# qingpingmo/OCN

Measured on AMD Instinct MI355X. Metric: candidate-edges/sec (CN predictor fwd), ogbl-collab shape, higher is better.
Workload: dtype f32

## Files before the change

include/ocn_hip.h:

```cpp
#ifndef OCN_HIP_H
#define OCN_HIP_H

#include <stdint.h>

#ifdef __cplusplus
extern "C" {
#endif

#define OCN_ABI_VERSION 9
#define OCN_EINVAL (-1)
#define OCN_ECAP   (-2)

#define OCN_ST_CAP  1
#define OCN_ST_SCAN 2
#define OCN_SCAN_POISON (-1)

#define OCN_F_CN1 1u
#define OCN_F_CN2 2u

int ocn_abi_version(void);

int64_t ocn_scan_workspace_bytes(int64_t n);

int ocn_zero_regions(void* const* ptrs, const int64_t* bytes, int32_t n, void* stream);
// ... 25 lines not shown
                    int64_t B, int64_t* order_out, int64_t* inv_out, int64_t* ranges, int64_t* prefix,
                    void* workspace, void* stream);

int ocn_scan_i32(const int32_t* in, int64_t n, int64_t* out, void* workspace, void* stream);

int ocn_cn_flags(const int64_t* rowptrA, const int32_t* colA,
                 const int64_t* rowptrT1, const int32_t* colT1,
                 const int64_t* rowptrT2, const int32_t* colT2,
                 const uint32_t* bitmapT1 , int64_t bm1_stride_words,
                 const uint32_t* bitmapT2 , int64_t bm_stride_words,
                 const int64_t* src, const int64_t* dst, const int64_t* order, int64_t B,
                 int64_t n_cols, const int64_t* off, uint8_t* flags, int64_t flags_cap,
                 uint64_t* hist , int32_t* cnt1, int32_t* cnt2,
                 int32_t* status, uint64_t* rec , int32_t* gcost , void* stream);
int ocn_cn_flags_rec(const int64_t* rowptrA, const int32_t* colA,
                     const int64_t* rowptrT1, const int32_t* colT1,
                     const int64_t* rowptrT2, const int32_t* colT2,
                     const uint32_t* bitmapT1 , int64_t bm1_stride_words,
                     const uint32_t* bitmapT2 , int64_t bm_stride_words,
                     const int64_t* src, const int64_t* dst, const int64_t* order, int64_t B,
                     int64_t n_cols, const int64_t* off, uint8_t* flags, int64_t flags_cap,
                     uint64_t* hist , int32_t* cnt1, int32_t* cnt2,
                     int32_t* status, uint64_t* rec , int32_t* gcost , void* stream);

int32_t ocn_walk_chunk(void);
int ocn_cn_walk_flags(const int64_t* rowptrA, const int32_t* colA, const int64_t* nds ,
                      const int64_t* src, const int64_t* dst, const int64_t* order, int64_t B,
                      const int64_t* chunk_off, const int64_t* rev_off , const int64_t* off,
                      int64_t max_row_len ,
                      uint8_t* flags, int32_t* wc, int64_t flags_cap,
                      uint64_t* hist , int32_t* cnt1, int32_t* cnt2,
                      int32_t* status, void* stream);

int ocn_neighbor_degree_sum(const int64_t* rowptr, const int32_t* col, int64_t n_rows, int64_t* out,
                            void* stream);
int ocn_walk_rev_offsets(const int64_t* rowptrA, const int64_t* nds, const int64_t* src, const int64_t* dst,
                         const int64_t* order, int64_t B, int64_t* out , void* workspace,
                         void* stream);

int32_t ocn_walk_prep_max_batch(void);
int ocn_walk_prep(const int64_t* rowptrA, const int64_t* nds , const int64_t* src, const int64_t* dst,
                  int64_t B, int32_t min_share, int64_t* order, int64_t* off, int64_t* chunk_off,
                  int64_t* rev_off , int32_t* g_head , int64_t* g_item_off ,
                  int32_t* g_active , int32_t* meta, int32_t* cnt1,
                  int32_t* cnt2, int32_t* status, int32_t* scal, void* stream);
int ocn_cn_walk_group(const int64_t* rowptrA, const int32_t* colA, const int64_t* src, const int64_t* dst,
// ... 332 lines not shown
```

ocn_amd/_lib.py:

```python
from __future__ import annotations

import ctypes
import glob
import os
import subprocess
from ctypes import c_float, c_int32, c_int64, c_void_p

_HERE = os.path.dirname(os.path.abspath(__file__))
_ROOT = os.path.dirname(_HERE)
LIB_PATH = os.environ.get("OCN_LIB_PATH", os.path.join(_HERE, "libocn_hip.so"))
CSRC = os.path.join(_HERE, "csrc")
INCLUDE = os.path.join(_ROOT, "include")

_P = c_void_p
ABI_VERSION = 9
SIGNATURES = {
    "ocn_abi_version": (c_int32, []),
    "ocn_scan_workspace_bytes": (c_int64, [c_int64]),
    "ocn_zero_regions": (c_int32, [_P, _P, c_int32, _P]),
    "ocn_check_edges": (c_int32, [_P, _P, c_int64, c_int64, c_int64, _P, _P]),
    "ocn_edge_offsets": (c_int32, [_P, _P, c_int64, _P, _P, _P]),
    "ocn_class_order": (c_int32, [_P, _P, _P, c_int64, _P, _P, _P, _P, _P, _P]),
    "ocn_scan_i32": (c_int32, [_P, c_int64, _P, _P, _P]),
    "ocn_order_workspace_bytes": (c_int64, [c_int64]),
    "ocn_order_by_node": (c_int32, [_P, c_int64, c_int64, _P, _P, _P]),
    "ocn_order_by_node_finish": (c_int32, [_P, c_int64, c_int64, _P, _P, _P]),
    "ocn_order_by_node_finish_rec": (c_int32, [_P, _P, _P, _P, c_int64, c_int64, _P, _P, _P, _P]),
    "ocn_batch_prep": (c_int32, [_P, _P, c_int64, _P, _P, c_int64, _P, _P, _P, c_int32, _P]),
    "ocn_cn_flags": (c_int32, [_P, _P, _P, _P, _P, _P, _P, c_int64, _P, c_int64, _P, _P, _P, c_int64, c_int64, _P, _P, c_int64, _P,
                               _P, _P, _P, _P, _P, _P]),
    "ocn_cn_flags_rec": (c_int32, [_P, _P, _P, _P, _P, _P, _P, c_int64, _P, c_int64, _P, _P, _P, c_int64, c_int64, _P, _P, c_int64, _P,
                                   _P, _P, _P, _P, _P, _P]),
    "ocn_chunk_offsets": (c_int32, [_P, _P, _P, _P, c_int64, _P, _P, _P]),
    "ocn_walk_chunk": (c_int32, []),
    "ocn_cn_walk_flags": (c_int32, [_P, _P, _P, _P, _P, _P, c_int64, _P, _P, _P, c_int64, _P, _P, c_int64, _P, _P, _P,
                                    _P, _P]),
    "ocn_neighbor_degree_sum": (c_int32, [_P, _P, c_int64, _P, _P]),
    "ocn_walk_prep_max_batch": (c_int32, []),
    "ocn_cn_flags_small_graph_cols": (c_int32, []),
    "ocn_cn_flags_pair_min_batch": (c_int64, [c_int64]),
    "ocn_walk_prep": (c_int32, [_P, _P, _P, _P, c_int64, c_int32, _P, _P, _P, _P, _P, _P, _P, _P, _P, _P, _P, _P, _P]),
    "ocn_cn_walk_group": (c_int32, [_P, _P, _P, _P, _P, c_int64, _P, _P, _P, _P, _P, _P, _P, c_int64, _P, _P, _P, _P]),
    "ocn_walk_rev_offsets": (c_int32, [_P, _P, _P, _P, _P, c_int64, _P, _P, _P]),
    "ocn_cn_weights_cn5": (c_int32, [_P, c_int64, _P, _P, c_int32, _P, _P]),
    "ocn_cn5_column_stats": (c_int32, [_P, c_int64, _P, _P]),
    "ocn_cn_colsum_workspace_bytes": (c_int64, [c_int64, c_int64]),
    "ocn_cn_colsum_exact": (c_int32, [_P, _P, _P, c_int64, _P, _P, _P, _P, c_int64, _P, c_int64, _P, _P, _P, _P, _P, _P, _P]),
    "ocn_cn_weights_cn7": (c_int32, [_P, c_int64, c_float, _P, _P, _P]),
    "ocn_cn_gather": (c_int32, [_P, _P, _P, _P, _P, c_int64, _P, _P, _P, _P, _P, c_int32, c_int64, _P, _P, _P, _P, _P,
                                _P, _P, _P, _P, _P]),
    "ocn_cn8_pool": (c_int32, [_P, _P, _P, _P, _P, _P, _P, c_int64, _P, c_int64, _P, _P, _P, c_int64, c_int64, _P, c_int32, _P, _P,
                               _P, _P, _P, _P]),
    "ocn_cn_pool_frozen": (c_int32, [_P, _P, _P, _P, _P, _P, _P, c_int64, _P, c_int64, _P, _P, _P, c_int64, c_int64, _P, _P, c_int32, _P,
                                     _P, _P, _P, _P, _P]),
    "ocn_cn_attribution": (c_int32, [_P, _P, _P, _P, c_int64, _P, _P, _P, c_int64, _P, _P, c_int32, _P, _P, _P, _P, _P]),
# ... 202 lines not shown
```

ocn_amd/csrc/cn_flags.hip:

```cpp
#include "common.h"


__device__ __forceinline__ bool sampled_has(const int32_t* samp, const int32_t* __restrict__ row, i64 n,
                                            int32_t key) {
  int lo = 0, hi = OCN_WAVE;
  while (lo < hi) {
    const int mid = (lo + hi) >> 1;
    if (samp[mid] <= key) lo = mid + 1; else hi = mid;
  }
  if (lo == 0) return false;
  const int s = lo - 1;
  const i64 p0 = ((i64)s * n) >> 6, p1 = ((i64)(s + 1) * n) >> 6;
  return sorted_has(row + p0, p1 - p0, key);
}

#define T1_CAP 1024

#define LH_MAX_COLS 8192

__device__ __forceinline__ i64 wave_uniform(i64 v) {
  const unsigned lo = __builtin_amdgcn_readfirstlane((unsigned)(u64)v), hi = __builtin_amdgcn_readfirstlane((unsigned)((u64)v >> 32));
  return (i64)(((u64)hi << 32) | lo);
}
__device__ __forceinline__ bool lanes_have(int32_t t, int32_t key) {
  int pos = 0;
#pragma unroll
  for (int step = OCN_WAVE / 2; step > 0; step >>= 1)
    if (__shfl(t, pos + step - 1, OCN_WAVE) < key) pos += step;
  return __shfl(t, pos, OCN_WAVE) == key;
}

template <bool HAS_T2, bool LH, bool RECIN, int NS>
__global__ __launch_bounds__(OCN_BLOCK) void cn_flags_kernel(
    const i64* __restrict__ rowptrA, const int32_t* __restrict__ colA,
    const i64* __restrict__ rowptrT1, const int32_t* __restrict__ colT1,
    const i64* __restrict__ rowptrT2, const int32_t* __restrict__ colT2,
    const unsigned* __restrict__ bmT1, i64 bm1_stride, const unsigned* __restrict__ bmT2, i64 bm_stride,
    const i64* __restrict__ src, const i64* __restrict__ dst, const i64* __restrict__ order, i64 B,
    i64 n_cols, const i64* __restrict__ off, uint8_t* __restrict__ flags, i64 cap,
    u64* __restrict__ hist, int32_t* __restrict__ cnt1, int32_t* __restrict__ cnt2,
    int32_t* __restrict__ status, u64* rec, int32_t* __restrict__ gcost) {
  constexpr int GPB = OCN_WPB, SPB = GPB * NS;
  constexpr int T1_PART = T1_CAP / NS, T2_PART = OCN_WAVE / NS;
  static_assert(NS == 1 || (NS == 2 && !LH), "slot pairs: large-graph forms only");
  __shared__ int s_cost[2][GPB];
  __shared__ int32_t s_t1[GPB][T1_CAP];
  __shared__ int32_t s_t2[GPB][OCN_WAVE];
  extern __shared__ __attribute__((aligned(16))) u64 s_hist[];
  const int gl = threadIdx.x % OCN_WAVE, g = __builtin_amdgcn_readfirstlane(threadIdx.x / OCN_WAVE);
  if (blockIdx.x == 0 && threadIdx.x == 0) status_raise(status, off[B], cap);
  const bool void_batch = off[B] < 0;
  if (LH) {
    for (i64 c = threadIdx.x; c < n_cols; c += OCN_BLOCK) s_hist[c] = 0ull;
    __syncthreads();
  }
  int par = 0;
  for (i64 e0 = (i64)blockIdx.x * SPB; e0 < B; e0 += (i64)gridDim.x * SPB, par ^= 1) {
    i64 slot[NS];
    bool act[NS];
    i64 e[NS], i[NS], j[NS], a0[NS], da[NS], b0[NS], db[NS], c0[NS], dc[NS], base[NS];
    const unsigned* bm_row[NS];
    const unsigned* bm1_row[NS];
#pragma unroll
    for (int s = 0; s < NS; ++s) {
// ... 17 lines not shown
#pragma unroll
            for (int q = 0; q < 4; ++q)
              w[q] = (u64)(unsigned)__builtin_amdgcn_readlane((int)(unsigned)recw, 4 * s + q) |
                     ((u64)(unsigned)__builtin_amdgcn_readlane((int)(unsigned)(recw >> 32), 4 * s + q) << 32);
          }
          e[s] = wave_uniform((i64)w[0]);
          i[s] = wave_uniform((i64)(w[1] & 0xffffffffull)); j[s] = wave_uniform((i64)(w[1] >> 32));
          a0[s] = wave_uniform((i64)(w[2] & ((1ull << REC_LEN_SHIFT) - 1))); da[s] = wave_uniform((i64)(w[2] >> REC_LEN_SHIFT));
          base[s] = wave_uniform((i64)w[3]);
        } else {
          e[s] = order ? order[slot[s]] : slot[s];
          i[s] = src[e[s]]; j[s] = dst[e[s]];
          a0[s] = rowptrA[i[s]]; da[s] = rowptrA[i[s] + 1] - a0[s];
          base[s] = off[e[s]];
        }
        if (bmT1) bm1_row[s] = bmT1 + j[s] * bm1_stride;
        else { b0[s] = rowptrT1[j[s]]; db[s] = rowptrT1[j[s] + 1] - b0[s]; }
        if (HAS_T2) {
          if (bmT2) bm_row[s] = bmT2 + j[s] * bm_stride;
          if (rowptrT2 && (LH || !bmT2)) { c0[s] = rowptrT2[j[s]]; dc[s] = rowptrT2[j[s] + 1] - c0[s]; }
        }
        if (void_batch) { da[s] = 0; db[s] = 0; dc[s] = 0; base[s] = 0; }
      }
    bool t1_reg[NS], t1_lds[NS], t2_full[NS], t2_lds[NS];
    int t1_at[NS], t2_at[NS];
    int32_t t1[NS];
#pragma unroll
    for (int s = 0; s < NS; ++s) {
      const int o = (s + 1) % NS;
      const bool whole1 = NS == 1 || db[o] <= OCN_WAVE;
      t1_reg[s] = db[s] <= OCN_WAVE; t1_lds[s] = db[s] <= (whole1 ? T1_CAP : T1_PART);
      t1_at[s] = whole1 ? 0 : s * T1_PART;
      t1[s] = 0x7fffffff;
      if (t1_reg[s]) { if (gl < db[s]) t1[s] = colT1[b0[s] + gl]; }
      else if (t1_lds[s])
        for (i64 q = gl; q < db[s]; q += OCN_WAVE) s_t1[g][t1_at[s] + q] = colT1[b0[s] + q];
    }
#pragma unroll
    for (int s = 0; s < NS; ++s) {
      const int o = (s + 1) % NS;
      t2_full[s] = HAS_T2 && rowptrT2 && dc[s] == n_cols;
      const bool whole2 = NS == 1 || (HAS_T2 && rowptrT2 && dc[o] == n_cols) || dc[o] == 0;
      t2_lds[s] = whole2 || dc[s] <= T2_PART;
      t2_at[s] = whole2 ? 0 : s * T2_PART;
      if (HAS_T2 && !t2_full[s] && !bmT2 && t2_lds[s]) {
        if (dc[s] > OCN_WAVE) s_t2[g][gl] = colT2[c0[s] + (((i64)gl * dc[s]) >> 6)];
        else if (gl < dc[s]) s_t2[g][t2_at[s] + gl] = colT2[c0[s] + gl];
      }
    }
    wave_lds_sync();
    bool fits[NS];
    int c1[NS], c2[NS];
    i64 da_max = da[0];
#pragma unroll
    for (int s = 0; s < NS; ++s) {
      fits[s] = base[s] + da[s] <= cap;
      c1[s] = c2[s] = 0;
      if (s > 0 && da[s] > da_max) da_max = da[s];
    }
    const bool same = NS > 1 && i[0] == i[NS - 1];
    for (i64 p0 = 0; p0 < da_max; p0 += OCN_WAVE) {
      const i64 p = p0 + gl;
      bool in[NS], f1[NS], f2[NS];
      int32_t k[NS];
      unsigned w2[NS];
#pragma unroll
      for (int s = 0; s < NS; ++s) {
        in[s] = p < da[s];
        if (s > 0 && same) k[s] = k[0];
        else k[s] = in[s] ? colA[a0[s] + p] : 0;
      }
#pragma unroll
      for (int s = 0; s < NS; ++s) {
        w2[s] = 0;
        if (HAS_T2 && bmT2 && !t2_full[s] && in[s]) w2[s] = bm_row[s][k[s] >> 5];
      }
#pragma unroll
      for (int s = 0; s < NS; ++s) {
        if (bmT1) f1[s] = in[s] && ((bm1_row[s][k[s] >> 5] >> (k[s] & 31)) & 1u);
        else if (t1_reg[s]) f1[s] = lanes_have(t1[s], k[s]) && in[s];
        else f1[s] = in[s] && (t1_lds[s] ? sorted_has(&s_t1[g][t1_at[s]], db[s], k[s]) : sorted_has(colT1 + b0[s], db[s], k[s]));
      }
#pragma unroll
      for (int s = 0; s < NS; ++s) {
        f2[s] = false;
        if (HAS_T2 && in[s]) {
          if (t2_full[s]) f2[s] = true;
          else if (bmT2) f2[s] = (w2[s] >> (k[s] & 31)) & 1u;
          else if (!t2_lds[s]) f2[s] = sorted_has(colT2 + c0[s], dc[s], k[s]);
          else f2[s] = dc[s] > OCN_WAVE ? sampled_has(&s_t2[g][0], colT2 + c0[s], dc[s], k[s]) : sorted_has(&s_t2[g][t2_at[s]], dc[s], k[s]);
        }
        if (fits[s] && in[s]) flags[base[s] + p] = (uint8_t)((f1[s] ? OCN_F_CN1 : 0u) | (f2[s] ? OCN_F_CN2 : 0u));
      }
      if (NS > 1 && same) {
        u64 inc = 0;
#pragma unroll
        for (int s = 0; s < NS; ++s) inc += (u64)f1[s] | ((u64)f2[s] << HF_BITS) | ((u64)(f1[s] | f2[s]) << (2 * HF_BITS));
        if (inc) atomicAdd(hist + 2 * (i64)k[0], inc);
      } else {
#pragma unroll
        for (int s = 0; s < NS; ++s)
          if (f1[s] | f2[s]) {
            const u64 inc = (u64)f1[s] | ((u64)f2[s] << HF_BITS) | (1ull << (2 * HF_BITS));
            if (LH) atomicAdd(s_hist + k[s], inc); else atomicAdd(hist + 2 * (i64)k[s], inc);
          }
      }
#pragma unroll
      for (int s = 0; s < NS; ++s) {
        c1[s] += __popcll(__ballot(f1[s]));
        c2[s] += __popcll(__ballot(f2[s]));
// ... 39 lines not shown
      const u64 v = s_hist[c];
      if (v) atomicAdd(hist + 2 * c, v);
    }
  }
}

extern "C" {

int32_t ocn_cn_flags_small_graph_cols(void) { return LH_MAX_COLS; }

static int64_t g_flags_pair_min_batch = 32768;

int64_t ocn_cn_flags_pair_min_batch(int64_t min_rows) {
  const int64_t prev = g_flags_pair_min_batch;
  if (min_rows >= 0) g_flags_pair_min_batch = min_rows;
  return prev;
}

static int cn_flags_launch(const int64_t* rowptrA, const int32_t* colA, const int64_t* rowptrT1,
                           const int32_t* colT1, const int64_t* rowptrT2, const int32_t* colT2,
                           const uint32_t* bitmapT1, int64_t bm1_stride_words, const uint32_t* bitmapT2, int64_t bm_stride_words,
                           const int64_t* src, const int64_t* dst, const int64_t* order, int64_t B,
                           int64_t n_cols, const int64_t* off, uint8_t* flags, int64_t flags_cap, uint64_t* hist,
                           int32_t* cnt1, int32_t* cnt2, int32_t* status, uint64_t* rec, int32_t* gcost, bool rec_in, void* stream) {
  if (B < 0 || flags_cap < 0 || B > (int64_t)HF_MASK) return OCN_EINVAL;
  if (B == 0) return 0;
  if (!rowptrA || (!rowptrT1 && !bitmapT1) || !src || !dst || !off || !hist || !cnt1 || !status) return OCN_EINVAL;
  if (rec_in && (!rec || !order)) return OCN_EINVAL;
  if ((bitmapT1 && bm1_stride_words * 32 < n_cols) || (bitmapT2 && bm_stride_words * 32 < n_cols)) return OCN_EINVAL;
  constexpr int GPB = OCN_WPB;
  hipStream_t st = (hipStream_t)stream;
  const bool lh = n_cols > 0 && n_cols <= LH_MAX_COLS;
  const size_t lds = lh ? (size_t)n_cols * sizeof(u64) : 0;
  const bool pairs = !lh && B >= g_flags_pair_min_batch;
  const int spb = pairs ? 2 * GPB : GPB;
  const int grid = lh ? grid_for((B + GPB - 1) / GPB, 256 * 3) : grid_for((B + spb - 1) / spb);
  if (lh) {
    static bool raised_dev[64] = {};
    int devid = 0;
    if (hipGetDevice(&devid) != hipSuccess || devid < 0 || devid >= 64) return OCN_EINVAL;
    bool& raised = raised_dev[devid];
    if (!raised) {
      const void* fns[4] = {(const void*)cn_flags_kernel<true, true, false, 1>, (const void*)cn_flags_kernel<false, true, false, 1>,
                            (const void*)cn_flags_kernel<true, true, true, 1>, (const void*)cn_flags_kernel<false, true, true, 1>};
      for (const void* fn : fns) {
        hipError_t e1 = hipFuncSetAttribute(fn, hipFuncAttributeMaxDynamicSharedMemorySize, LH_MAX_COLS * (int)sizeof(u64));
        if (e1 != hipSuccess) return (int)e1;
      }
      raised = true;
    }
  }
#define CN_FLAGS_ARGS(T2P, T2C)                                                                      \
  (const i64*)rowptrA, colA, (const i64*)rowptrT1, colT1, (const i64*)(T2P), (T2C),                   \
      (const unsigned*)bitmapT1, (i64)bm1_stride_words, (const unsigned*)bitmapT2, (i64)bm_stride_words, (const i64*)src, \
      (const i64*)dst, (const i64*)order, (i64)B, (i64)n_cols, (const i64*)off, flags, (i64)flags_cap, \
      (u64*)hist, cnt1, cnt2, status, (u64*)rec, gcost
#define CN_FLAGS_LAUNCH(T2, LHV, RI, NSV, T2P, T2C)                                                   \
  hipLaunchKernelGGL((cn_flags_kernel<T2, LHV, RI, NSV>), dim3(grid), dim3(OCN_BLOCK), (LHV) ? lds : 0, st, CN_FLAGS_ARGS(T2P, T2C))
#define CN_FLAGS_PICK(T2, T2P, T2C)                                                                   \
  do {                                                                                                \
    if (lh) { if (rec_in) CN_FLAGS_LAUNCH(T2, true, true, 1, T2P, T2C); else CN_FLAGS_LAUNCH(T2, true, false, 1, T2P, T2C); }   \
    else if (pairs) { if (rec_in) CN_FLAGS_LAUNCH(T2, false, true, 2, T2P, T2C); else CN_FLAGS_LAUNCH(T2, false, false, 2, T2P, T2C); }   \
    else { if (rec_in) CN_FLAGS_LAUNCH(T2, false, true, 1, T2P, T2C); else CN_FLAGS_LAUNCH(T2, false, false, 1, T2P, T2C); }    \
  } while (0)
  if (!rowptrT2 && bitmapT2 && lh) return OCN_EINVAL;
  if (rowptrT2 || bitmapT2) CN_FLAGS_PICK(true, rowptrT2, colT2);
  else CN_FLAGS_PICK(false, nullptr, (const int32_t*)nullptr);
#undef CN_FLAGS_PICK
#undef CN_FLAGS_LAUNCH
  return launch_status();
}

int ocn_cn_flags(const int64_t* rowptrA, const int32_t* colA, const int64_t* rowptrT1,
                 const int32_t* colT1, const int64_t* rowptrT2, const int32_t* colT2,
                 const uint32_t* bitmapT1, int64_t bm1_stride_words, const uint32_t* bitmapT2, int64_t bm_stride_words,
                 const int64_t* src, const int64_t* dst, const int64_t* order, int64_t B,
                 int64_t n_cols, const int64_t* off, uint8_t* flags, int64_t flags_cap, uint64_t* hist,
                 int32_t* cnt1, int32_t* cnt2, int32_t* status, uint64_t* rec, int32_t* gcost, void* stream) {
  return cn_flags_launch(rowptrA, colA, rowptrT1, colT1, rowptrT2, colT2, bitmapT1, bm1_stride_words, bitmapT2, bm_stride_words,
                         src, dst, order, B, n_cols, off, flags, flags_cap, hist, cnt1, cnt2, status, rec, gcost, false, stream);
}

int ocn_cn_flags_rec(const int64_t* rowptrA, const int32_t* colA, const int64_t* rowptrT1,
                     const int32_t* colT1, const int64_t* rowptrT2, const int32_t* colT2,
                     const uint32_t* bitmapT1, int64_t bm1_stride_words, const uint32_t* bitmapT2, int64_t bm_stride_words,
                     const int64_t* src, const int64_t* dst, const int64_t* order, int64_t B,
                     int64_t n_cols, const int64_t* off, uint8_t* flags, int64_t flags_cap, uint64_t* hist,
                     int32_t* cnt1, int32_t* cnt2, int32_t* status, uint64_t* rec, int32_t* gcost, void* stream) {
  return cn_flags_launch(rowptrA, colA, rowptrT1, colT1, rowptrT2, colT2, bitmapT1, bm1_stride_words, bitmapT2, bm_stride_words,
                         src, dst, order, B, n_cols, off, flags, flags_cap, hist, cnt1, cnt2, status, rec, gcost, true, stream);
}

}
```

ocn_amd/ops.py:

```python
from __future__ import annotations

import ctypes
import os
from typing import Optional, Tuple

import torch
from torch import Tensor

from . import _lib
from ._lib import check, ptr, stream_ptr

FLAGS_NOSYNC_LIMIT = 1 << 30
validate_indices = True
stage_timer = None
LN_WIDTHS = (16, 32, 64, 128, 256, 512)
a1_bitmap_max_bytes = int(os.environ.get("OCN_A1_BITMAP_MAX_BYTES", 64 << 20))
a2_bitmap_max_bytes = 16 << 30
skip_zero_rows = True
skip_zero_min_share = 0.15
skip_zero_backoff = 32
skip_zero_min_batch = 4096
walk_two_sided = True
walk_share_min = 2
sort_edges_min_batch = 4096
heavy_first = os.environ.get("OCN_HEAVY_FIRST", "1") != "0"
sched_segment = int(os.environ.get("OCN_SCHED_SEG", 0))
overlap_depth = int(os.environ.get("OCN_OVERLAP_DEPTH", 4))
overlap_depth_small = int(os.environ.get("OCN_OVERLAP_DEPTH_SMALL", 8))
overlap_small_batch = 4096
overlap_deep_max_batch = int(os.environ.get("OCN_OVERLAP_DEEP_MAX_BATCH", 1 << 30))
shard_reduce_in_finish = {"0": False, "1": True}.get(os.environ.get("OCN_REDUCE_IN_FINISH", ""), None)
_overlap_active = False
phase_a_extras = os.environ.get("OCN_PHASE_A_EXTRAS", "1") != "0"
phase_a_pool = os.environ.get("OCN_PHASE_A_POOL", "1") != "0"
graph_loops = os.environ.get("OCN_GRAPH_LOOPS", "0") == "1"
graph_loops_min_batches_per_set = 6
overlap_min_batch = 2048
overlap_streams = os.environ.get("OCN_ONE_STREAM", "0") != "1"
share_full_rows = True
deterministic_backward = os.environ.get("OCN_ATOMIC_BACKWARD", "0") != "1"


def loop_depth(batch) -> int:
    if batch is None or batch > overlap_deep_max_batch:
        return 2
    return max(2, int(overlap_depth_small if batch <= overlap_small_batch else overlap_depth))


# ... 206 lines not shown


def _nds_arg(nds: Optional[Tensor], n: int) -> Optional[Tensor]:
    if nds is not None and _req(nds, torch.int64, "nds", 1).numel() != n:
        raise ValueError("nds does not match the adjacency")
    return nds


def _flag_capacity(B: int, max_deg_a: int, off: Tensor) -> int:
    bound = B * max(int(max_deg_a), 0)
    return bound if bound <= FLAGS_NOSYNC_LIMIT else _total(off[-1])


def _cn_operands(rowptrA, colA, t1, t2, bm1, bm2, src, dst, order, B: int, n_cols: int):
    return (ptr(rowptrA), ptr(colA), ptr(t1[0]), ptr(t1[1]), ptr(t2[0]), ptr(t2[1]),
            ptr(bm1), bm1.shape[1] if bm1 is not None else 0, ptr(bm2), bm2.shape[1] if bm2 is not None else 0,
            ptr(src), ptr(dst), ptr(order), B, n_cols)


@_on_device
def cn_flags(rowptrA: Tensor, colA: Tensor, t1: Optional[Tuple[Tensor, Tensor]],
             t2: Optional[Tuple[Tensor, Tensor]], src: Tensor, dst: Tensor, n_cols: int, max_deg_a: int,
             walk: bool = False, t2_bitmap: Optional[Tensor] = None, wsd=None, nds: Optional[Tensor] = None,
             t1_bitmap: Optional[Tensor] = None, rec: Optional[Tensor] = None, sched: Optional[Tensor] = None):
    dev = src.device
    _req(rowptrA, torch.int64, "rowptrA", 1); _req(colA, torch.int32, "colA", 1)
    has_t2 = not walk and t2 is not None
    if not walk:
        *csr1, rows = _t_of_flag_pass(t1, t1_bitmap, "T1", n_cols)
        if t2 is None and t2_bitmap is not None:
            raise ValueError("t2_bitmap does not match the T2 adjacency")
        *csr2, _ = (None, None, None) if not has_t2 else _t_of_flag_pass(
            t2, t2_bitmap, "T2", n_cols, like=rows, col_deferred=True, rowptr_optional=t2[0] is None and n_cols > small_graph_cols())
    B = _batch_ids(src, dst, hist=True)
    _mark("begin")
    if walk and 0 < B <= int(_lib.lib().ocn_walk_prep_max_batch()) and walk_share_min > 0:
        return _cn_flags_walk_small(rowptrA, colA, src, dst, n_cols, max_deg_a, wsd, nds)
    want_order = B >= sort_edges_min_batch
    n_src = rowptrA.numel() - 1
    order = buf(wsd, "order", B, torch.int64, dev) if want_order else None
    ows = (buf(wsd, "order_ws", int(_lib.lib().ocn_order_workspace_bytes(n_src)) // 8 + 1, torch.int64, dev, zero_init=True)
           if want_order else None)
    off = buf(wsd, "off", B + 1, torch.int64, dev)
    sws = _ws(B, dev, wsd)
    hist = buf(wsd, "hist", (n_cols, 2), torch.int64, dev)
    cnt1 = buf(wsd, "cnt1", B, torch.int32, dev)
    cnt2 = buf(wsd, "cnt2", B, torch.int32, dev) if (walk or has_t2) else None
# ... 18 lines not shown
        check(_lib.lib().ocn_order_by_node_finish(ptr(src), B, n_src, ptr(order), ptr(ows), stream_ptr()),
              "ocn_order_by_node_finish")
    cap = _flag_capacity(B, max_deg_a, off)
    flags = buf(wsd, "flags", max(cap, 1), torch.uint8, dev)
    wc = buf(wsd, "wc", max(cap, 1), torch.int32, dev) if walk else None
    chunk_off = rev_off = None
    if walk:
        nds = _nds_arg(nds if walk_two_sided else None, n_src)
        chunk_off = buf(wsd, "chunk_off", B + 1, torch.int64, dev)
        cws = _ws(B, dev, wsd)
        check(_lib.lib().ocn_chunk_offsets(ptr(rowptrA), ptr(nds), ptr(src), ptr(order), B, ptr(chunk_off), ptr(cws),
                                           stream_ptr()), "ocn_chunk_offsets")
        if nds is not None:
            rev_off = buf(wsd, "rev_off", B + 1, torch.int64, dev)
            check(_lib.lib().ocn_walk_rev_offsets(ptr(rowptrA), ptr(nds), ptr(src), ptr(dst), ptr(order), B,
                                                  ptr(rev_off), ptr(cws), stream_ptr()), "ocn_walk_rev_offsets")
    _mark("cn_prep")
    if walk:
        check(_lib.lib().ocn_cn_walk_flags(ptr(rowptrA), ptr(colA), ptr(nds), ptr(src), ptr(dst), ptr(order), B,
                                           ptr(chunk_off), ptr(rev_off), ptr(off), int(max_deg_a), ptr(flags),
                                           ptr(wc), cap, ptr(hist), ptr(cnt1), ptr(cnt2), ptr(status),
                                           stream_ptr()), "ocn_cn_walk_flags")
    else:
        check((_lib.lib().ocn_cn_flags_rec if rec_in else _lib.lib().ocn_cn_flags)(
            *_cn_operands(rowptrA, colA, csr1, csr2, t1_bitmap, t2_bitmap, src, dst, order, B, n_cols), ptr(off), ptr(flags), cap,
            ptr(hist), ptr(cnt1), ptr(cnt2), ptr(status), ptr(rec), ptr(sched), stream_ptr()), "ocn_cn_flags")
    _mark("cn_flags")
    return order, off, flags, wc, hist, cnt1, cnt2, status, scal


def _cn_flags_walk_small(rowptrA, colA, src, dst, n_cols, max_deg_a, wsd, nds):
    dev, B = src.device, src.numel()
    l = _lib.lib()
    nds = _nds_arg(nds if walk_two_sided else None, rowptrA.numel() - 1)
    order = buf(wsd, "order", B, torch.int64, dev)
    off = buf(wsd, "off", B + 1, torch.int64, dev)
    chunk_off = buf(wsd, "chunk_off", B + 1, torch.int64, dev)
    rev_off = buf(wsd, "rev_off", B + 1, torch.int64, dev) if nds is not None else None
    g_head = buf(wsd, "g_head", B + 1, torch.int32, dev)
    g_item_off = buf(wsd, "g_item_off", B + 1, torch.int64, dev)
    g_active = buf(wsd, "g_active", B, torch.int32, dev)
    meta = buf(wsd, "walk_meta", 4, torch.int32, dev)
    hist = buf(wsd, "hist", (n_cols, 2), torch.int64, dev)
    cnt1 = buf(wsd, "cnt1", B, torch.int32, dev)
    cnt2 = buf(wsd, "cnt2", B, torch.int32, dev)
    status = buf(wsd, "status", 4, torch.int32, dev, zero_init=True)
    scal = buf(wsd, "scal", 4, torch.int32, dev)
    check(l.ocn_walk_prep(ptr(rowptrA), ptr(nds), ptr(src), ptr(dst), B, int(walk_share_min), ptr(order), ptr(off),
                          ptr(chunk_off), ptr(rev_off), ptr(g_head), ptr(g_item_off), ptr(g_active), ptr(meta), ptr(cnt1),
# ... 1659 lines not shown
```

ocn_amd/sparse.py:

```python
from __future__ import annotations

from typing import List, Optional, Tuple

import torch
from torch import Tensor

from . import ops


class _Storage:
    def __init__(self, owner: "SparseTensor"):
        self._o = owner

    def row(self) -> Tensor:
        return self._o._row64()

    def col(self) -> Tensor:
        return self._o._col.to(torch.int64)

    def rowptr(self) -> Tensor:
        return self._o._rowptr

    def rowcount(self) -> Tensor:
        return self._o._rowptr[1:] - self._o._rowptr[:-1]

    def value(self) -> Optional[Tensor]:
        return self._o._value

    def has_value(self) -> bool:
        return self._o._value is not None


class SparseTensor:
    def __new__(cls, row=None, rowptr=None, col=None, value=None, sparse_sizes=None, *a, **k):
        cn = getattr(row, "_ocn_lazy_cn", None)
        if cn is not None:
            if getattr(col, "_ocn_lazy_cn", None) is not cn or (value is not None and getattr(value, "_ocn_lazy_cn", None) is not cn):
                raise NotImplementedError("row / col / value of different deferred common-neighbour matrices")
            if sparse_sizes is not None and tuple(int(v) for v in sparse_sizes) != tuple(cn.shape):
                raise ValueError(f"sparse_sizes {tuple(sparse_sizes)} != {tuple(cn.shape)} of the deferred matrix")
            return cn.batch()
        return super().__new__(cls)

    def __init__(self, row: Optional[Tensor] = None, rowptr: Optional[Tensor] = None,
                 col: Optional[Tensor] = None, value: Optional[Tensor] = None,
                 sparse_sizes: Optional[Tuple[int, int]] = None, is_sorted: bool = False,
                 trust_data: bool = False):
        assert col is not None and (row is not None or rowptr is not None)
        if sparse_sizes is None:
            n_rows = (int(row.max()) + 1 if row.numel() else 0) if rowptr is None else rowptr.numel() - 1
            n_cols = int(col.max()) + 1 if col.numel() else 0
            sparse_sizes = (n_rows, n_cols)
        self._sizes = (int(sparse_sizes[0]), int(sparse_sizes[1]))
        if rowptr is None and value is None and not is_sorted and col.is_cuda:
            rowptr, col = ops.coo_to_csr(row.to(torch.int64), col.to(torch.int64), self._sizes[0], self._sizes[1],
                                         check_range=not trust_data)
# ... 194 lines not shown
        return self._bitmap

    def neighbor_degree_sum(self) -> Tensor:
        if self._nds is None:
            self._nds = ops.neighbor_degree_sum(self._rowptr, self._col)
            self._published("nds")
        else:
            self._await("nds")
        return self._nds

    def product_bit_rows(self) -> Optional[Tensor]:
        self.complete()
        if self._bitmap is not None:
            self._await("bitmap")
        return self._bitmap

    def probed_bit_rows(self, dst: Tensor, row_lengths: bool = False) -> Optional[Tensor]:
        if self.rows_on_demand() and not ops._overlap_active and not (row_lengths and self._sizes[1] <= ops.small_graph_cols()):
            a_rp, a_col, b_rp, b_col = self._lazy
            ops.spgemm_bit_rows(a_rp, a_col, b_rp, b_col, self._sizes[1], dst, self._done, self._bitmap)
            return self._bitmap
        return self.product_bit_rows()

    def rows_on_demand(self) -> bool:
        return getattr(self, "_lazy", None) is not None

    def complete(self) -> None:
        if self.rows_on_demand():
            self._complete()

    def warm(self, walk: bool = False) -> None:
        self.max_rowcount()
        if walk:
            self.neighbor_degree_sum()
        else:
            self.bit_rows()

    def to_device(self, device, non_blocking: bool = False) -> "SparseTensor":
        out = SparseTensor(rowptr=self._rowptr.to(device, non_blocking=non_blocking),
                           col=self._col.to(device, non_blocking=non_blocking),
                           value=None if self._value is None else self._value.to(device, non_blocking=non_blocking),
                           sparse_sizes=self._sizes)
        out._maxdeg = self._maxdeg
        return out

    def to(self, device, non_blocking: bool = False):
        return self.to_device(device, non_blocking)

    def cuda(self):
        return self.to_device("cuda")

    def cpu(self):
        return self.to_device("cpu")

    def set_value(self, value: Optional[Tensor]) -> "SparseTensor":
        out = SparseTensor(rowptr=self._rowptr, col=self._col, value=value, sparse_sizes=self._sizes)
        out._row_cache, out._maxdeg = self._row_cache, self._maxdeg
        return out

    def fill_value(self, v: float, dtype=torch.float32) -> "SparseTensor":
        return self.set_value(torch.full((self.nnz(),), v, dtype=dtype, device=self._col.device))

    def fill_value_(self, v: float, dtype=torch.float32) -> "SparseTensor":
        self._value = torch.full((self.nnz(),), v, dtype=dtype, device=self._col.device)
        return self

    def coalesce(self, reduce: str = "sum") -> "SparseTensor":
        n = max(self._sizes[1], 1)
        key = self._row64() * n + self._col.to(torch.int64)
        if self._value is None:
            ukey = torch.unique_consecutive(key)
            val = None
        else:
            ukey, inv = torch.unique_consecutive(key, return_inverse=True)
            val = torch.zeros(ukey.numel(), dtype=self._value.dtype, device=key.device).index_add_(0, inv, self._value)
        return SparseTensor(row=torch.div(ukey, n, rounding_mode="floor"), col=ukey % n, value=val,
                            sparse_sizes=self._sizes, is_sorted=True, trust_data=True)

    def to_symmetric(self, reduce: str = "sum") -> "SparseTensor":
        r, c = self._row64(), self._col.to(torch.int64)
        if self._value is None and self._col.is_cuda and self._sizes[0] == self._sizes[1]:
            rowptr, col = ops.coo_to_csr(r, c, self._sizes[0], self._sizes[1], symmetrize=True, dedupe=True, check_range=False)
            return SparseTensor(rowptr=rowptr, col=col, sparse_sizes=self._sizes)
        v = None if self._value is None else torch.cat([self._value, self._value])
        return SparseTensor(row=torch.cat([r, c]), col=torch.cat([c, r]), value=v,
                            sparse_sizes=self._sizes, trust_data=True).coalesce(reduce)

    def t(self) -> "SparseTensor":
        if getattr(self, "_t_cache", None) is None:
            r, c = self._row64(), self._col.to(torch.int64)
            self._t_cache = SparseTensor(row=c, col=r, value=self._value, sparse_sizes=(self._sizes[1], self._sizes[0]),
                                         trust_data=True)
        return self._t_cache

    def __getitem__(self, idx: Tensor) -> "SparseTensor":
        idx = idx.to(torch.int64)
        start = self._rowptr[idx]
        deg = self._rowptr[idx + 1] - start
        optr = torch.zeros(idx.numel() + 1, dtype=torch.int64, device=idx.device)
        torch.cumsum(deg, 0, out=optr[1:])
        total = int(optr[-1])
        row = torch.repeat_interleave(torch.arange(idx.numel(), device=idx.device), deg, output_size=total)
        pos = torch.arange(total, device=idx.device) - optr[:-1][row] + start[row]
        return SparseTensor(rowptr=optr, col=self._col[pos],
                            value=None if self._value is None else self._value[pos],
                            sparse_sizes=(idx.numel(), self._sizes[1]))

    def to_dense(self) -> Tensor:
        d = torch.zeros(self._sizes, device=self._col.device)
# ... 55 lines not shown
        self.sp = sp
        self.is_product = is_product

    @property
    def shape(self):
        return tuple(self.sp._sizes)

    def __matmul__(self, other: "CooView") -> "CooView":
        a, b = self.sp, other.sp
        if a._sizes[1] != b._sizes[0]:
            raise ValueError("shape mismatch in sparse @ sparse")
        n, m = a._sizes[0], b._sizes[1]
        if (ops.lazy_product_rows and torch.is_grad_enabled() and a._rowptr.is_cuda and m > ops.small_graph_cols()
                and 0 < n * ((m + 31) // 32) * 4 <= ops.a2_bitmap_max_bytes and m <= ops.spgemm_max_cols()):
            return CooView(SparseTensor._lazy_product(a, b), is_product=True)
        rowptr, col, bitmap = ops.spgemm_pattern(a._rowptr, a._col, b._rowptr, b._col, b._sizes[1], defer_fill=True)
        if callable(col):
            out = SparseTensor._deferred_product(rowptr, col, bitmap, (a._sizes[0], b._sizes[1]))
        else:
            out = SparseTensor(rowptr=rowptr, col=col, sparse_sizes=(a._sizes[0], b._sizes[1]))
            out._bitmap = bitmap
        if bitmap is not None:
            out._published("bitmap")
        return CooView(out, is_product=True)

    def to_torch(self) -> Tensor:
        sp = self.sp
        v = sp._value if sp._value is not None else torch.ones(sp.nnz(), device=sp.device())
        return torch.sparse_coo_tensor(torch.stack([sp._row64(), sp._col.to(torch.int64)]), v, sp._sizes)
```

ocn_amd/update.py:

```python
from __future__ import annotations

import warnings
from typing import List, Optional, Tuple

import torch
import torch.nn as nn
from torch import Tensor

from . import ops
from .sparse import SparseTensor


_WORDS = {"insert_edges": ("new_edges", "take new entries"), "remove_edges": ("edges", "give up entries")}


def _check_args(fn: str, adj: SparseTensor, edges: Tensor, adj2: Optional[SparseTensor]) -> int:
    arg, verb = _WORDS[fn]
    if not isinstance(adj, SparseTensor) or (adj2 is not None and not isinstance(adj2, SparseTensor)):
        raise ValueError(f"{fn}: adj (and adj2) must be SparseTensor objects")
    if adj.has_value() or (adj2 is not None and not adj2.rows_on_demand() and adj2.has_value()):
        raise ValueError(f"{fn}: a valued adjacency cannot {verb} (pattern matrices only)")
    n, m = adj.sparse_sizes()
    if n != m:
        raise ValueError(f"{fn}: adj is {n} x {m}, not square")
    if adj2 is not None and tuple(adj2.sparse_sizes()) != (n, n):
        raise ValueError(f"{fn}: adj2 is {tuple(adj2.sparse_sizes())}, adj {(n, n)}")
    if not isinstance(edges, Tensor) or edges.dtype != torch.int64 or edges.dim() != 2 or edges.shape[0] != 2:
        raise ValueError(f"{fn}: {arg} must be an int64 tensor of shape [2, E]")
    if edges.device != adj.device():
        raise ValueError(f"{fn}: {arg} on {edges.device}, adj on {adj.device()}")
    return n


def _retire(adj2: SparseTensor) -> None:
    adj2._lazy = adj2._done = None
    adj2._rowptr_v = None
    adj2._col_v = adj2._col_thunk = None
    adj2._bitmap = None
    adj2._row_cache = adj2._maxdeg = adj2._nds = None
    adj2._ready = {}


def _cpu_pair(row: Tensor, col: Tensor, n: int, with_product: bool):
    adj_new = SparseTensor(row=row, col=col, sparse_sizes=(n, n), is_sorted=True, trust_data=True)
    if not with_product:
        return adj_new, None
    a = torch.sparse_coo_tensor(torch.stack([row, col]), torch.ones(row.numel(), dtype=torch.float64), (n, n))
    with warnings.catch_warnings():
        warnings.simplefilter("ignore", UserWarning)
        p = torch.sparse.mm(a, a).coalesce()
    pr, pc = p.indices()
    return adj_new, SparseTensor(row=pr, col=pc, sparse_sizes=(n, n), is_sorted=True, trust_data=True)


def _delta_csr(fn: str, edges: Tensor, n: int, undirected: bool) -> Tuple[Tensor, Tensor]:
    try:
        return ops.coo_to_csr(edges[0], edges[1], n, n, symmetrize=undirected, dedupe=True)
    except IndexError as e:
# ... 318 lines not shown
```

ocn_amd/utils.py:

```python
from __future__ import annotations

from typing import Optional, Tuple

import torch
from torch import Tensor

from . import ops
from .sparse import SparseTensor


class PermIterator:

    def __init__(self, device, size, bs, training=True) -> None:
        self.bs = bs
        self.training = training
        self.idx = torch.randperm(size, device=device) if training else torch.arange(size, device=device)

    def __len__(self):
        return (self.idx.shape[0] + (self.bs - 1) * (not self.training)) // self.bs

    def __iter__(self):
        self.ptr = 0
        return self

# ... 64 lines not shown
    _sched_ready = False
    sharded, shard_group = False, None

    def __init__(self, adj: SparseTensor, t1: Optional[SparseTensor], t2: Optional[SparseTensor],
                 tarei: Tensor, walk: bool = False, ws: Optional[dict] = None):
        self.src, self.dst = _endpoints(tarei)
        for t in (t1, t2):
            if t is not None and t.sparse_sizes() != adj.sparse_sizes():
                raise ValueError("adjoverlap: adjacency sizes differ")
        if walk and adj.size(0) != adj.size(1):
            raise ValueError("get_cn1_cn2 needs a square adjacency")
        self.adj, self.walk, self.t2 = adj, walk, t2
        self.ws = ws
        self.B = self.src.numel()
        self.N = adj.size(1)
        ops.check_edges(self.src, self.dst, adj.size(0), adj.size(0) if walk else t1.size(0))
        self.rec = None if (walk or self.B == 0) else ops.buf(ws, "rec", (self.B, 4), torch.int64, self.src.device)
        self.sched = (ops.buf(ws, "sched", 2 * ((self.B + 3) // 4), torch.int32, self.src.device)
                      if (self.rec is not None and ops.heavy_first and self.B >= ops.sort_edges_min_batch) else None)
        csr2 = bm2 = None
        if t2 is not None and not walk:
            bm2 = t2.probed_bit_rows(self.dst, row_lengths=True)
            csr2 = (t2.rowptr_formed(), t2._col if (t2.col_materialized() or bm2 is None) else None)
        (self.order, self.off, self.flags, self.wc, self.hist, self.cnt1, self.cnt2, self.status, self.scal) = ops.cn_flags(
            adj._rowptr, adj._col, None if walk else (t1._rowptr, t1._col), csr2, self.src, self.dst, self.N,
            adj.max_rowcount(), walk=walk, t2_bitmap=bm2, wsd=ws,
            nds=adj.neighbor_degree_sum() if (walk and ops.walk_two_sided) else None,
            t1_bitmap=None if walk else t1.bit_rows(), rec=self.rec, sched=self.sched)
        self._hist_live = True

    @classmethod
    def from_materialized(cls, adj: SparseTensor, cn1: SparseTensor, cn2: SparseTensor, tarei: Tensor,
                          ws: Optional[dict] = None) -> "CNState":
        st = cls.__new__(cls)
        st.adj, st.ws = adj, ws
        st.src, st.dst = _endpoints(tarei)
        st.B, st.N = st.src.numel(), adj.size(1)
        dev = st.src.device
        if tuple(cn1.sizes()) != (st.B, st.N) or tuple(cn2.sizes()) != (st.B, st.N):
            raise ValueError("cn1 / cn2 must be [B, N] with B = tar_ei.shape[1], N = adj.size(1)")
        ops.check_edges(st.src, st.dst, adj.size(0), adj.size(0))
        st.off = ops.edge_offsets(adj._rowptr, st.src)
        total = int(st.off[-1])
        st.flags = torch.zeros(max(total, 1), dtype=torch.uint8, device=dev)
        rows_sel = adj[st.src]
        r_s, c_s, _ = rows_sel.coo()
        key_s = r_s * st.N + c_s
        v2 = cn2.storage.value()
        st.walk = bool(v2 is not None and v2.numel() and bool((v2 != 1).any()))
        st.wc = torch.zeros(max(total, 1), dtype=torch.int32, device=dev) if st.walk else None
        for bit, m in ((1, cn1), (2, cn2)):
# ... 302 lines not shown
        raise NotImplementedError("calresadj / neighbour sampling are outside the cn5/cn7 path")
    return CNBatch(adj1, adj2, tarei)


def adjoverlap_3hop(adj: SparseTensor, adj2: SparseTensor, tarei: Tensor, undirected: bool = True) -> CNBatch:
    _check_hop3(adj, adj2, tarei)
    return CNBatch(adj, adj2, tarei, "hop3", undirected=bool(undirected))


def get_cn1_cn2(adj: SparseTensor, tedge: Tensor) -> Tuple[CNBatch, CNBatch]:
    return CNBatch(adj, None, tedge, "walk1"), CNBatch(adj, None, tedge, "walk2")


def block_matrix_multiply(spadj: SparseTensor, block_size: int, fold_quirk: bool = False) -> SparseTensor:
    n = spadj.size(0)
    if spadj.size(1) != n:
        raise ValueError("block_matrix_multiply needs a square adjacency")
    if n <= ops.dense_adj2_max_nodes and block_size > 0 and block_size % 32 == 0 and spadj._col.is_cuda:
        rowptr, col, bits = ops.dense_block_adj2(spadj._rowptr, spadj._col, n, int(block_size), fold=fold_quirk)
        out = SparseTensor(rowptr=rowptr, col=col, sparse_sizes=(n, n))
        if not fold_quirk:
            out._bitmap = bits
            out._published("bitmap")
        return out
    if fold_quirk:
        raise NotImplementedError("fold_quirk needs the dense block route (n <= ops.dense_adj2_max_nodes, block_size % 32 == 0)")
    return SparseTensor.from_torch_sparse_coo_tensor(
        spadj.to_torch_sparse_coo_tensor() @ spadj.to_torch_sparse_coo_tensor(), False)


def sparse_tensor_multiply(spadj: SparseTensor, block_size: int = 1024) -> SparseTensor:
    return block_matrix_multiply(spadj, block_size, fold_quirk=bool(ops.adj2_fold_quirk))
```

Before: 176.3 million.

## Skip T2 membership probes when dst neighbors src and T2 is the square of adj

Adds a cover shortcut: when T2 is certified to be adj squared and adj is symmetric, every neighbor k of i lies in row j of T2 whenever j is itself a neighbor of i. The kernel checks whether j is in row i of A (with a ballot for short rows, or a sampled search for rows up to a cap) and, if so, marks every f2 as true without reading the bitmap or CSR. Python-side bookkeeping tracks the square relation and symmetry so the kernel only takes this path when it is valid. The cost is an extra sampled load and ballot per edge, a one-time symmetry check against the transpose, and more kernel complexity.

Measured after the change: 179.5 million, median of 6. 1.02x the previous value.

```diff
diff --git a/include/ocn_hip.h b/include/ocn_hip.h
--- a/include/ocn_hip.h
+++ b/include/ocn_hip.h
@@ -71,6 +71,16 @@
                      int64_t n_cols, const int64_t* off, uint8_t* flags, int64_t flags_cap,
                      uint64_t* hist , int32_t* cnt1, int32_t* cnt2,
                      int32_t* status, uint64_t* rec , int32_t* gcost , void* stream);
+int ocn_cn_flags_cover(const int64_t* rowptrA, const int32_t* colA,
+                       const int64_t* rowptrT1, const int32_t* colT1,
+                       const int64_t* rowptrT2, const int32_t* colT2,
+                       const uint32_t* bitmapT1 , int64_t bm1_stride_words,
+                       const uint32_t* bitmapT2 , int64_t bm_stride_words,
+                       const int64_t* src, const int64_t* dst, const int64_t* order, int64_t B,
+                       int64_t n_cols, const int64_t* off, uint8_t* flags, int64_t flags_cap,
+                       uint64_t* hist , int32_t* cnt1, int32_t* cnt2,
+                       int32_t* status, uint64_t* rec , int32_t* gcost ,
+                       int32_t rec_in, int32_t t2_cover, void* stream);
 
 int32_t ocn_walk_chunk(void);
 int ocn_cn_walk_flags(const int64_t* rowptrA, const int32_t* colA, const int64_t* nds ,
diff --git a/ocn_amd/_lib.py b/ocn_amd/_lib.py
--- a/ocn_amd/_lib.py
+++ b/ocn_amd/_lib.py
@@ -31,6 +31,8 @@
                                _P, _P, _P, _P, _P, _P]),
     "ocn_cn_flags_rec": (c_int32, [_P, _P, _P, _P, _P, _P, _P, c_int64, _P, c_int64, _P, _P, _P, c_int64, c_int64, _P, _P, c_int64, _P,
                                    _P, _P, _P, _P, _P, _P]),
+    "ocn_cn_flags_cover": (c_int32, [_P, _P, _P, _P, _P, _P, _P, c_int64, _P, c_int64, _P, _P, _P, c_int64, c_int64, _P, _P, c_int64, _P,
+                                     _P, _P, _P, _P, _P, c_int32, c_int32, _P]),
     "ocn_chunk_offsets": (c_int32, [_P, _P, _P, _P, c_int64, _P, _P, _P]),
     "ocn_walk_chunk": (c_int32, []),
     "ocn_cn_walk_flags": (c_int32, [_P, _P, _P, _P, _P, _P, c_int64, _P, _P, _P, c_int64, _P, _P, c_int64, _P, _P, _P,
diff --git a/ocn_amd/csrc/cn_flags.hip b/ocn_amd/csrc/cn_flags.hip
--- a/ocn_amd/csrc/cn_flags.hip
+++ b/ocn_amd/csrc/cn_flags.hip
@@ -30,6 +30,7 @@
   return __shfl(t, pos, OCN_WAVE) == key;
 }
 
+#define COVER_MAX_ROW 4096
 template <bool HAS_T2, bool LH, bool RECIN, int NS>
 __global__ __launch_bounds__(OCN_BLOCK) void cn_flags_kernel(
     const i64* __restrict__ rowptrA, const int32_t* __restrict__ colA,
@@ -39,7 +40,7 @@
     const i64* __restrict__ src, const i64* __restrict__ dst, const i64* __restrict__ order, i64 B,
     i64 n_cols, const i64* __restrict__ off, uint8_t* __restrict__ flags, i64 cap,
     u64* __restrict__ hist, int32_t* __restrict__ cnt1, int32_t* __restrict__ cnt2,
-    int32_t* __restrict__ status, u64* rec, int32_t* __restrict__ gcost) {
+    int32_t* __restrict__ status, u64* rec, int32_t* __restrict__ gcost, int cover) {
   constexpr int GPB = OCN_WPB, SPB = GPB * NS;
   constexpr int T1_PART = T1_CAP / NS, T2_PART = OCN_WAVE / NS;
   static_assert(NS == 1 || (NS == 2 && !LH), "slot pairs: large-graph forms only");
@@ -103,6 +104,15 @@
         }
         if (void_batch) { da[s] = 0; db[s] = 0; dc[s] = 0; base[s] = 0; }
       }
+    const bool same = NS > 1 && i[0] == i[NS - 1];
+    bool seek[NS], skip2[NS];
+    int32_t smp[NS];
+#pragma unroll
+    for (int s = 0; s < NS; ++s) {
+      seek[s] = HAS_T2 && cover && da[s] > OCN_WAVE && da[s] <= COVER_MAX_ROW;
+      smp[s] = 0x7fffffff;
+      if (seek[s]) smp[s] = (s > 0 && same) ? smp[0] : colA[a0[s] + (((i64)gl * da[s]) >> 6)];
+    }
     bool t1_reg[NS], t1_lds[NS], t2_full[NS], t2_lds[NS];
     int t1_at[NS], t2_at[NS];
     int32_t t1[NS];
@@ -121,6 +131,7 @@
     for (int s = 0; s < NS; ++s) {
       const int o = (s + 1) % NS;
       t2_full[s] = HAS_T2 && rowptrT2 && dc[s] == n_cols;
+      skip2[s] = t2_full[s];
       const bool whole2 = NS == 1 || (HAS_T2 && rowptrT2 && dc[o] == n_cols) || dc[o] == 0;
       t2_lds[s] = whole2 || dc[s] <= T2_PART;
       t2_at[s] = whole2 ? 0 : s * T2_PART;
@@ -129,6 +140,16 @@
         else if (gl < dc[s]) s_t2[g][t2_at[s] + gl] = colT2[c0[s] + gl];
       }
     }
+#pragma unroll
+    for (int s = 0; s < NS; ++s)
+      if (seek[s]) {
+        const int nle = __popcll(__ballot(smp[s] <= (int32_t)j[s]));
+        if (nle > 0) {
+          const i64 q0 = ((i64)(nle - 1) * da[s]) >> 6, q1 = ((i64)nle * da[s]) >> 6;
+          const int32_t v = q0 + gl < q1 ? colA[a0[s] + q0 + gl] : -1;
+          skip2[s] = skip2[s] || __ballot(v == (int32_t)j[s]) != 0;
+        }
+      }
     wave_lds_sync();
     bool fits[NS];
     int c1[NS], c2[NS];
@@ -139,7 +160,6 @@
       c1[s] = c2[s] = 0;
       if (s > 0 && da[s] > da_max) da_max = da[s];
     }
-    const bool same = NS > 1 && i[0] == i[NS - 1];
     for (i64 p0 = 0; p0 < da_max; p0 += OCN_WAVE) {
       const i64 p = p0 + gl;
       bool in[NS], f1[NS], f2[NS];
@@ -151,10 +171,15 @@
         if (s > 0 && same) k[s] = k[0];
         else k[s] = in[s] ? colA[a0[s] + p] : 0;
       }
+      if (HAS_T2 && cover && p0 == 0) {
+#pragma unroll
+        for (int s = 0; s < NS; ++s)
+          if (da[s] <= OCN_WAVE) skip2[s] = skip2[s] || __ballot(in[s] && k[s] == (int32_t)j[s]) != 0;
+      }
 #pragma unroll
       for (int s = 0; s < NS; ++s) {
         w2[s] = 0;
-        if (HAS_T2 && bmT2 && !t2_full[s] && in[s]) w2[s] = bm_row[s][k[s] >> 5];
+        if (HAS_T2 && bmT2 && !skip2[s] && in[s]) w2[s] = bm_row[s][k[s] >> 5];
       }
 #pragma unroll
       for (int s = 0; s < NS; ++s) {
@@ -166,7 +191,7 @@
       for (int s = 0; s < NS; ++s) {
         f2[s] = false;
         if (HAS_T2 && in[s]) {
-          if (t2_full[s]) f2[s] = true;
+          if (skip2[s]) f2[s] = true;
           else if (bmT2) f2[s] = (w2[s] >> (k[s] & 31)) & 1u;
           else if (!t2_lds[s]) f2[s] = sorted_has(colT2 + c0[s], dc[s], k[s]);
           else f2[s] = dc[s] > OCN_WAVE ? sampled_has(&s_t2[g][0], colT2 + c0[s], dc[s], k[s]) : sorted_has(&s_t2[g][t2_at[s]], dc[s], k[s]);
@@ -252,7 +277,7 @@
                            const uint32_t* bitmapT1, int64_t bm1_stride_words, const uint32_t* bitmapT2, int64_t bm_stride_words,
                            const int64_t* src, const int64_t* dst, const int64_t* order, int64_t B,
                            int64_t n_cols, const int64_t* off, uint8_t* flags, int64_t flags_cap, uint64_t* hist,
-                           int32_t* cnt1, int32_t* cnt2, int32_t* status, uint64_t* rec, int32_t* gcost, bool rec_in, void* stream) {
+                           int32_t* cnt1, int32_t* cnt2, int32_t* status, uint64_t* rec, int32_t* gcost, bool rec_in, bool cover, void* stream) {
   if (B < 0 || flags_cap < 0 || B > (int64_t)HF_MASK) return OCN_EINVAL;
   if (B == 0) return 0;
   if (!rowptrA || (!rowptrT1 && !bitmapT1) || !src || !dst || !off || !hist || !cnt1 || !status) return OCN_EINVAL;
@@ -284,7 +309,7 @@
   (const i64*)rowptrA, colA, (const i64*)rowptrT1, colT1, (const i64*)(T2P), (T2C),                   \
       (const unsigned*)bitmapT1, (i64)bm1_stride_words, (const unsigned*)bitmapT2, (i64)bm_stride_words, (const i64*)src, \
       (const i64*)dst, (const i64*)order, (i64)B, (i64)n_cols, (const i64*)off, flags, (i64)flags_cap, \
-      (u64*)hist, cnt1, cnt2, status, (u64*)rec, gcost
+      (u64*)hist, cnt1, cnt2, status, (u64*)rec, gcost, (int)cover
 #define CN_FLAGS_LAUNCH(T2, LHV, RI, NSV, T2P, T2C)                                                   \
   hipLaunchKernelGGL((cn_flags_kernel<T2, LHV, RI, NSV>), dim3(grid), dim3(OCN_BLOCK), (LHV) ? lds : 0, st, CN_FLAGS_ARGS(T2P, T2C))
 #define CN_FLAGS_PICK(T2, T2P, T2C)                                                                   \
@@ -308,7 +333,7 @@
                  int64_t n_cols, const int64_t* off, uint8_t* flags, int64_t flags_cap, uint64_t* hist,
                  int32_t* cnt1, int32_t* cnt2, int32_t* status, uint64_t* rec, int32_t* gcost, void* stream) {
   return cn_flags_launch(rowptrA, colA, rowptrT1, colT1, rowptrT2, colT2, bitmapT1, bm1_stride_words, bitmapT2, bm_stride_words,
-                         src, dst, order, B, n_cols, off, flags, flags_cap, hist, cnt1, cnt2, status, rec, gcost, false, stream);
+                         src, dst, order, B, n_cols, off, flags, flags_cap, hist, cnt1, cnt2, status, rec, gcost, false, false, stream);
 }
 
 int ocn_cn_flags_rec(const int64_t* rowptrA, const int32_t* colA, const int64_t* rowptrT1,
@@ -318,7 +343,19 @@
                      int64_t n_cols, const int64_t* off, uint8_t* flags, int64_t flags_cap, uint64_t* hist,
                      int32_t* cnt1, int32_t* cnt2, int32_t* status, uint64_t* rec, int32_t* gcost, void* stream) {
   return cn_flags_launch(rowptrA, colA, rowptrT1, colT1, rowptrT2, colT2, bitmapT1, bm1_stride_words, bitmapT2, bm_stride_words,
-                         src, dst, order, B, n_cols, off, flags, flags_cap, hist, cnt1, cnt2, status, rec, gcost, true, stream);
-}
-
-}
+                         src, dst, order, B, n_cols, off, flags, flags_cap, hist, cnt1, cnt2, status, rec, gcost, true, false, stream);
+}
+
+int ocn_cn_flags_cover(const int64_t* rowptrA, const int32_t* colA, const int64_t* rowptrT1,
+                       const int32_t* colT1, const int64_t* rowptrT2, const int32_t* colT2,
+                       const uint32_t* bitmapT1, int64_t bm1_stride_words, const uint32_t* bitmapT2, int64_t bm_stride_words,
+                       const int64_t* src, const int64_t* dst, const int64_t* order, int64_t B,
+                       int64_t n_cols, const int64_t* off, uint8_t* flags, int64_t flags_cap, uint64_t* hist,
+                       int32_t* cnt1, int32_t* cnt2, int32_t* status, uint64_t* rec, int32_t* gcost, int32_t rec_in,
+                       int32_t t2_cover, void* stream) {
+  return cn_flags_launch(rowptrA, colA, rowptrT1, colT1, rowptrT2, colT2, bitmapT1, bm1_stride_words, bitmapT2, bm_stride_words,
+                         src, dst, order, B, n_cols, off, flags, flags_cap, hist, cnt1, cnt2, status, rec, gcost, rec_in != 0,
+                         t2_cover != 0 && (rowptrT2 || bitmapT2), stream);
+}
+
+}
diff --git a/ocn_amd/ops.py b/ocn_amd/ops.py
--- a/ocn_amd/ops.py
+++ b/ocn_amd/ops.py
@@ -24,6 +24,7 @@
 walk_share_min = 2
 sort_edges_min_batch = 4096
 heavy_first = os.environ.get("OCN_HEAVY_FIRST", "1") != "0"
+t2_cover = os.environ.get("OCN_T2_COVER", "1") != "0"
 sched_segment = int(os.environ.get("OCN_SCHED_SEG", 0))
 overlap_depth = int(os.environ.get("OCN_OVERLAP_DEPTH", 4))
 overlap_depth_small = int(os.environ.get("OCN_OVERLAP_DEPTH_SMALL", 8))
@@ -276,7 +277,8 @@
 def cn_flags(rowptrA: Tensor, colA: Tensor, t1: Optional[Tuple[Tensor, Tensor]],
              t2: Optional[Tuple[Tensor, Tensor]], src: Tensor, dst: Tensor, n_cols: int, max_deg_a: int,
              walk: bool = False, t2_bitmap: Optional[Tensor] = None, wsd=None, nds: Optional[Tensor] = None,
-             t1_bitmap: Optional[Tensor] = None, rec: Optional[Tensor] = None, sched: Optional[Tensor] = None):
+             t1_bitmap: Optional[Tensor] = None, rec: Optional[Tensor] = None, sched: Optional[Tensor] = None,
+             t2_certified: bool = False):
     dev = src.device
     _req(rowptrA, torch.int64, "rowptrA", 1); _req(colA, torch.int32, "colA", 1)
     has_t2 = not walk and t2 is not None
@@ -341,9 +343,10 @@
                                            ptr(wc), cap, ptr(hist), ptr(cnt1), ptr(cnt2), ptr(status),
                                            stream_ptr()), "ocn_cn_walk_flags")
     else:
-        check((_lib.lib().ocn_cn_flags_rec if rec_in else _lib.lib().ocn_cn_flags)(
+        check(_lib.lib().ocn_cn_flags_cover(
             *_cn_operands(rowptrA, colA, csr1, csr2, t1_bitmap, t2_bitmap, src, dst, order, B, n_cols), ptr(off), ptr(flags), cap,
-            ptr(hist), ptr(cnt1), ptr(cnt2), ptr(status), ptr(rec), ptr(sched), stream_ptr()), "ocn_cn_flags")
+            ptr(hist), ptr(cnt1), ptr(cnt2), ptr(status), ptr(rec), ptr(sched), int(rec_in),
+            int(bool(t2_certified) and has_t2 and t2_cover), stream_ptr()), "ocn_cn_flags")
     _mark("cn_flags")
     return order, off, flags, wc, hist, cnt1, cnt2, status, scal
 
diff --git a/ocn_amd/sparse.py b/ocn_amd/sparse.py
--- a/ocn_amd/sparse.py
+++ b/ocn_amd/sparse.py
@@ -32,6 +32,9 @@
 
 
 class SparseTensor:
+    _square_of: Optional["SparseTensor"] = None
+    _symmetric: Optional[bool] = None
+
     def __new__(cls, row=None, rowptr=None, col=None, value=None, sparse_sizes=None, *a, **k):
         cn = getattr(row, "_ocn_lazy_cn", None)
         if cn is not None:
@@ -272,6 +275,19 @@
             return self._bitmap
         return self.product_bit_rows()
 
+    def is_symmetric(self) -> bool:
+        if self._symmetric is None:
+            if self._sizes[0] != self._sizes[1]:
+                self._symmetric = False
+            else:
+                at = self.t()
+                self._symmetric = bool(torch.equal(self._rowptr, at._rowptr) and torch.equal(self._col, at._col))
+        return self._symmetric
+
+    def covers(self, adj: "SparseTensor") -> bool:
+        return (self._square_of is not None and self._square_of is adj and not self.rows_on_demand()
+                and adj.is_symmetric())
+
     def rows_on_demand(self) -> bool:
         return getattr(self, "_lazy", None) is not None
 
@@ -285,6 +301,8 @@
             self.neighbor_degree_sum()
         else:
             self.bit_rows()
+            if ops.t2_cover and self._rowptr.is_cuda:
+                self.is_symmetric()
 
     def to_device(self, device, non_blocking: bool = False) -> "SparseTensor":
         out = SparseTensor(rowptr=self._rowptr.to(device, non_blocking=non_blocking),
@@ -331,10 +349,13 @@
         r, c = self._row64(), self._col.to(torch.int64)
         if self._value is None and self._col.is_cuda and self._sizes[0] == self._sizes[1]:
             rowptr, col = ops.coo_to_csr(r, c, self._sizes[0], self._sizes[1], symmetrize=True, dedupe=True, check_range=False)
-            return SparseTensor(rowptr=rowptr, col=col, sparse_sizes=self._sizes)
-        v = None if self._value is None else torch.cat([self._value, self._value])
-        return SparseTensor(row=torch.cat([r, c]), col=torch.cat([c, r]), value=v,
-                            sparse_sizes=self._sizes, trust_data=True).coalesce(reduce)
+            out = SparseTensor(rowptr=rowptr, col=col, sparse_sizes=self._sizes)
+        else:
+            v = None if self._value is None else torch.cat([self._value, self._value])
+            out = SparseTensor(row=torch.cat([r, c]), col=torch.cat([c, r]), value=v,
+                               sparse_sizes=self._sizes, trust_data=True).coalesce(reduce)
+        out._symmetric = self._sizes[0] == self._sizes[1]
+        return out
 
     def t(self) -> "SparseTensor":
         if getattr(self, "_t_cache", None) is None:
@@ -436,6 +457,8 @@
             out._bitmap = bitmap
         if bitmap is not None:
             out._published("bitmap")
+        if a is b:
+            out._square_of = a
         return CooView(out, is_product=True)
 
     def to_torch(self) -> Tensor:
diff --git a/ocn_amd/update.py b/ocn_amd/update.py
--- a/ocn_amd/update.py
+++ b/ocn_amd/update.py
@@ -34,6 +34,7 @@
 
 def _retire(adj2: SparseTensor) -> None:
     adj2._lazy = adj2._done = None
+    adj2._square_of = None
     adj2._rowptr_v = None
     adj2._col_v = adj2._col_thunk = None
     adj2._bitmap = None
diff --git a/ocn_amd/utils.py b/ocn_amd/utils.py
--- a/ocn_amd/utils.py
+++ b/ocn_amd/utils.py
@@ -110,11 +110,12 @@
         if t2 is not None and not walk:
             bm2 = t2.probed_bit_rows(self.dst, row_lengths=True)
             csr2 = (t2.rowptr_formed(), t2._col if (t2.col_materialized() or bm2 is None) else None)
+        certified = bool(csr2 is not None and ops.t2_cover and t2.covers(adj))
         (self.order, self.off, self.flags, self.wc, self.hist, self.cnt1, self.cnt2, self.status, self.scal) = ops.cn_flags(
             adj._rowptr, adj._col, None if walk else (t1._rowptr, t1._col), csr2, self.src, self.dst, self.N,
             adj.max_rowcount(), walk=walk, t2_bitmap=bm2, wsd=ws,
             nds=adj.neighbor_degree_sum() if (walk and ops.walk_two_sided) else None,
-            t1_bitmap=None if walk else t1.bit_rows(), rec=self.rec, sched=self.sched)
+            t1_bitmap=None if walk else t1.bit_rows(), rec=self.rec, sched=self.sched, t2_certified=certified)
         self._hist_live = True
 
     @classmethod
@@ -463,6 +464,7 @@
         if not fold_quirk:
             out._bitmap = bits
             out._published("bitmap")
+            out._square_of = spadj
         return out
     if fold_quirk:
         raise NotImplementedError("fold_quirk needs the dense block route (n <= ops.dense_adj2_max_nodes, block_size % 32 == 0)")
```
